# graphdeco-inria/gaussian-splatting

Measured on AMD Instinct MI355X. Metric: Mpix/s forward (1 M Gaussians @1080p); train iters/s alongside, higher is better.
Workload: dtype f32; 1 GPU; configs[1] stand-in: 1M random Gaussians (SURVEY 8(d) generator, seed 0, s_med 0.012), 1920x1080 forward render, SH degree 3; P=1000000, visible=876281, num_rendered=7916318, tiles=8160, parallelism=one GPU, mode=single, render_fwd_variant=0, options=, frame_streams=1

## Files before the change

### gaussian-splatting_amd/csrc/preprocess.hip

```cpp
#include "gsr_internal.h"
#include "gsr_adam_math.h"
#include "gsr_frame.h"

namespace {

#ifndef GSR_PRE_OCC_FWD
#define GSR_PRE_OCC_FWD
#endif
#ifndef GSR_PRE_OCC_BWD
#ifdef GSR_SIMT_SHIM
#define GSR_PRE_OCC_BWD
#else
#define GSR_PRE_OCC_BWD __attribute__((amdgpu_waves_per_eu(2, 2)))
#endif
#endif

constexpr int SH_ROW = 52;

__device__ __forceinline__ void load_cam(const GsrCamDev& c, GsrCam& cam) {
    cam.W = c.W; cam.H = c.H; cam.gx = c.gx; cam.gy = c.gy;
    cam.focal_x = c.focal_x; cam.focal_y = c.focal_y; cam.limx = c.limx; cam.limy = c.limy;
    cam.scale_modifier = c.scale_modifier; cam.sh_degree = c.sh_degree; cam.M = c.M;
    cam.antialiasing = c.antialiasing; cam.tile_y0 = c.tile_y0; cam.tile_y1 = c.tile_y1; cam.snug = c.snug;
#pragma unroll
    for (int i = 0; i < 16; ++i) { cam.view[i] = c.view[i]; cam.proj[i] = c.proj[i]; }
#pragma unroll
    for (int i = 0; i < 3; ++i) cam.campos[i] = c.campos[i];
}

#ifdef GSR_SIMT_SHIM
__device__ __forceinline__ void fence_loaded12(float4 (&)[12]) {}
#else
typedef float gsr_v4f __attribute__((ext_vector_type(4)));
__device__ __forceinline__ void fence_loaded12(float4 (&v)[12]) {
    gsr_v4f r[12];
#pragma unroll
    for (int k = 0; k < 12; ++k) r[k] = (gsr_v4f){v[k].x, v[k].y, v[k].z, v[k].w};
    asm volatile("" : "+v"(r[0]), "+v"(r[1]), "+v"(r[2]), "+v"(r[3]), "+v"(r[4]), "+v"(r[5]), "+v"(r[6]), "+v"(r[7]), "+v"(r[8]),
                      "+v"(r[9]), "+v"(r[10]), "+v"(r[11]));
#pragma unroll
    for (int k = 0; k < 12; ++k) v[k] = make_float4(r[k].x, r[k].y, r[k].z, r[k].w);
    __builtin_amdgcn_sched_barrier(0);
}
#endif

__device__ __forceinline__ void wave_load_sh16(const float* __restrict__ shs, int64_t i0, int P, uint64_t rows, int lane,
                                               float* tile) {
    const float4* src = reinterpret_cast<const float4*>(shs + i0 * 48);
    float4 v[12];
#pragma unroll
    for (int it = 0; it < 12; ++it) {
        const int idx = it * 64 + lane;
        const int g = idx / 12;
        v[it] = src[(((rows >> g) & 1ull) && i0 + g < P) ? idx : 0];
    }
    fence_loaded12(v);
#pragma unroll
    for (int it = 0; it < 12; ++it) {
        const int idx = it * 64 + lane;
        const int g = idx / 12, part = idx - g * 12;
        *reinterpret_cast<float4*>(tile + g * SH_ROW + part * 4) = v[it];
    }
    __builtin_amdgcn_wave_barrier();
}
__device__ __forceinline__ void wave_issue_sh16(const float* __restrict__ shs, int64_t i0, int P, int lane, float4 (&reg)[12]) {
    const float4* src = reinterpret_cast<const float4*>(shs + i0 * 48);
#pragma unroll
    for (int it = 0; it < 12; ++it) {
        const int idx = it * 64 + lane;
        const int g = idx / 12;
        reg[it] = (i0 + g < P) ? src[idx] : make_float4(0.f, 0.f, 0.f, 0.f);
    }
}
__device__ __forceinline__ void wave_commit_sh16(const float4 (&reg)[12], uint64_t rows, int lane, float* tile) {
#pragma unroll
    for (int it = 0; it < 12; ++it) {
        const int idx = it * 64 + lane;
        const int g = idx / 12, part = idx - g * 12;
        if ((rows >> g) & 1ull) *reinterpret_cast<float4*>(tile + g * SH_ROW + part * 4) = reg[it];
    }
    __builtin_amdgcn_wave_barrier();
}
__device__ __forceinline__ void wave_store_sh16(float* __restrict__ dst_all, int64_t i0, int P, int lane, const float* tile) {
    float4* dst = reinterpret_cast<float4*>(dst_all + i0 * 48);
    __builtin_amdgcn_wave_barrier();
#pragma unroll
    for (int it = 0; it < 12; ++it) {
        const int idx = it * 64 + lane;
        const int g = idx / 12, part = idx - g * 12;
        if (i0 + g < P) dst[idx] = *reinterpret_cast<const float4*>(tile + g * SH_ROW + part * 4);
    }
    __builtin_amdgcn_wave_barrier();
}

constexpr int SPLIT_DC = 64 * 45;
__device__ __forceinline__ void wave_load_sh_split_dense(const float* __restrict__ dc, const float* __restrict__ rest, int64_t i0,
                                                         int P, uint64_t rows, int lane, float* tile) {
    const int nrow = (int)((P - i0) < 64 ? (P - i0) : 64);
    const float* src = rest + i0 * 45;
    const float* sdc = dc + i0 * 3;
    const int nrest = nrow * 45, ndc = nrow * 3;
    float4 v[12];
    bool ok[12];
#pragma unroll
    for (int it = 0; it < 12; ++it) {
        const int f = (it * 64 + lane) * 4;
        const int g0 = f / 45, g1 = (f + 3) / 45;
        const bool want = rows == ~0ull || ((((rows >> (g0 & 63)) | (rows >> (g1 & 63))) & 1ull) != 0);
        ok[it] = want && f + 3 < nrest;
        v[it] = *reinterpret_cast<const float4*>(src + (ok[it] ? f : 0));
    }
    const int fd = lane * 4;
    const bool okd = rows != 0ull && fd + 3 < ndc;
    const float4 vd = *reinterpret_cast<const float4*>(sdc + (okd ? fd : 0));
    fence_loaded12(v);
#pragma unroll
    for (int it = 0; it < 12; ++it) {
        const int f = (it * 64 + lane) * 4;
        *reinterpret_cast<float4*>(tile + (f < 64 * 45 ? f : 64 * 48 + lane * 4)) = v[it];
    }
    *reinterpret_cast<float4*>(tile + (fd < 64 * 3 ? SPLIT_DC + fd : 64 * 48 + lane * 4)) = vd;
    (void)ok; (void)okd;
    if (lane < (nrest & 3)) tile[(nrest & ~3) + lane] = src[(nrest & ~3) + lane];
    if (lane < (ndc & 3)) tile[SPLIT_DC + (ndc & ~3) + lane] = sdc[(ndc & ~3) + lane];
    __builtin_amdgcn_wave_barrier();
}
__device__ __forceinline__ void wave_store_sh_split_dense(float* __restrict__ d_dc, float* __restrict__ d_rest, int64_t i0, int P,
                                                          int lane, const float* tile) {
    const int nrow = (int)((P - i0) < 64 ? (P - i0) : 64);
    float* dst = d_rest + i0 * 45;
    const int nrest = nrow * 45;
    __builtin_amdgcn_wave_barrier();
#pragma unroll
    for (int it = 0; it < 12; ++it) {
        const int f = (it * 64 + lane) * 4;
        if (f + 3 < nrest) {
            *reinterpret_cast<float4*>(dst + f) = *reinterpret_cast<const float4*>(tile + f);
        } else if (f < nrest) {
            for (int c = 0; c < 3; ++c)
                if (f + c < nrest) dst[f + c] = tile[f + c];
        }
    }
    float* ddc = d_dc + i0 * 3;
    const int ndc = nrow * 3, fd = lane * 4;
    if (fd + 3 < ndc) {
        *reinterpret_cast<float4*>(ddc + fd) = *reinterpret_cast<const float4*>(tile + SPLIT_DC + fd);
    } else if (fd < ndc) {
        for (int c = 0; c < 3; ++c)
            if (fd + c < ndc) ddc[fd + c] = tile[SPLIT_DC + fd + c];
    }
    __builtin_amdgcn_wave_barrier();
}
template <bool SPLIT>
__global__ void __launch_bounds__(256) GSR_PRE_OCC_FWD
preprocess_fwd_kernel(GsrCamDev camd, int P, const float* __restrict__ means3D, const float* __restrict__ shs,
                      const float* __restrict__ colors_precomp, const float* __restrict__ opacities,
                      const float* __restrict__ scales, const float* __restrict__ rotations,
                      const float* __restrict__ cov3D_precomp, float4* __restrict__ splats,
                      uint2* __restrict__ rect, uint32_t* __restrict__ tiles, uint32_t* __restrict__ clamped_out,
                      uint32_t* __restrict__ keys, uint32_t* __restrict__ vals, int32_t* __restrict__ radii,
                      GsrFrameStatsDev fs) {
    __shared__ __attribute__((aligned(16))) float s_sh[4][64 * SH_ROW];
    GsrCam cam;
    load_cam(camd, cam);
    const int lane = threadIdx.x & 63, wv = threadIdx.x >> 6;
    float* tile = s_sh[wv];
    const float* dc = SPLIT ? camd.sh_dc : nullptr;
    const bool staged_sh = shs != nullptr && cam.M == 16;
    const bool speculative = (cam.tile_y1 - cam.tile_y0) * 4 >= cam.gy;
    GsrFrameAcc acc;
    for (int64_t i0 = ((int64_t)blockIdx.x * blockDim.x + threadIdx.x) - lane; i0 < P; i0 += (int64_t)gridDim.x * blockDim.x) {
        const int64_t i = i0 + lane;
        const bool in_range = i < P;
        GsrSplat sp;
        sp.radius = 0; sp.tiles = 0; sp.minx = sp.miny = sp.maxx = sp.maxy = 0; sp.depth = 0.f;
        float mean[3] = {0.f, 0.f, 0.f};
        bool vis = false;
        const bool spec_sh = staged_sh && speculative;
        float4 g_rot = make_float4(0.f, 0.f, 0.f, 0.f);
        float g_s[3] = {0.f, 0.f, 0.f}, g_op = 0.f;
        if (spec_sh) {
            float4 shreg[12];
            if (!SPLIT) wave_issue_sh16(shs, i0, P, lane, shreg);
            if (in_range) {
                mean[0] = means3D[i * 3 + 0]; mean[1] = means3D[i * 3 + 1]; mean[2] = means3D[i * 3 + 2];
                g_op = opacities[i];
                if (!cov3D_precomp) {
                    g_s[0] = scales[i * 3 + 0]; g_s[1] = scales[i * 3 + 1]; g_s[2] = scales[i * 3 + 2];
                    g_rot = reinterpret_cast<const float4*>(rotations)[i];
                }
            }
            if (SPLIT) wave_load_sh_split_dense(dc, shs, i0, P, ~0ull, lane, tile);
            else wave_commit_sh16(shreg, ~0ull, lane, tile);
        }
        if (in_range) {
            if (!spec_sh) {
                mean[0] = means3D[i * 3 + 0]; mean[1] = means3D[i * 3 + 1]; mean[2] = means3D[i * 3 + 2];
                g_op = opacities[i];
            }
            float cov[6];
            if (cov3D_precomp) {
#pragma unroll
                for (int k = 0; k < 6; ++k) cov[k] = cov3D_precomp[i * 6 + k];
            } else {
                if (!spec_sh) {
                    g_s[0] = scales[i * 3 + 0]; g_s[1] = scales[i * 3 + 1]; g_s[2] = scales[i * 3 + 2];
                    g_rot = reinterpret_cast<const float4*>(rotations)[i];
                }
                const float q[4] = {g_rot.x, g_rot.y, g_rot.z, g_rot.w};
                gsr_cov3d(g_s, cam.scale_modifier, q, cov);
            }
            vis = gsr_project(cam, mean, cov, g_op, sp);
        }
        const bool need_color = vis && sp.tiles > 0;
        if (staged_sh) {
            const uint64_t rows = __ballot(need_color);
            if (rows) {
                if (spec_sh) {  }
                else if (SPLIT) wave_load_sh_split_dense(dc, shs, i0, P, rows, lane, tile);
                else wave_load_sh16(shs, i0, P, rows, lane, tile);
            }
        }
        if (!in_range) continue;
        uint32_t clampbits = 0;
        float4 q0 = make_float4(0.f, 0.f, 0.f, 0.f), q1 = q0, q2 = q0;
        if (vis) {
            float rgb[3] = {0.f, 0.f, 0.f};
            if (!need_color) {
            } else if (colors_precomp) {
                rgb[0] = colors_precomp[i * 3 + 0]; rgb[1] = colors_precomp[i * 3 + 1]; rgb[2] = colors_precomp[i * 3 + 2];
            } else if (staged_sh) {
                if (SPLIT) gsr_sh_to_rgb_row(cam.sh_degree, 16, GsrShRowSplit{tile + SPLIT_DC + lane * 3, tile + lane * 45}, mean, cam.campos, rgb, clampbits);
                else gsr_sh_to_rgb_row(cam.sh_degree, 16, GsrShRowAligned{tile + lane * SH_ROW}, mean, cam.campos, rgb, clampbits);
            } else if (!SPLIT) {
                gsr_sh_to_rgb(cam.sh_degree, cam.M, shs + i * (int64_t)cam.M * 3, mean, cam.campos, rgb, clampbits);
            }
            q0 = make_float4(sp.px, sp.py, sp.conA, sp.conB);
            q1 = make_float4(sp.conC, sp.opacity, rgb[0], rgb[1]);
            q2 = make_float4(rgb[2], sp.depth, sp.tau, gsr_inv_depth(sp.depth));
        }
        const uint2 rc = make_uint2(sp.minx | (sp.maxx << 16), sp.miny | (sp.maxy << 16));
        splats[i * 4 + 0] = q0;
        splats[i * 4 + 1] = q1;
        splats[i * 4 + 2] = q2;
        splats[i * 4 + 3] = make_float4(__uint_as_float(rc.x), __uint_as_float(rc.y), 0.f, __uint_as_float(sp.tiles));
        rect[i] = rc;
        tiles[i] = sp.tiles;
        if (clamped_out) clamped_out[i] = clampbits;
        radii[i] = sp.radius;
        const uint32_t key = gsr_depth_key(sp.depth, sp.tiles != 0u, acc.ovf);
        keys[i] = key;
        vals[i] = (uint32_t)i;
        acc.add(key, sp.tiles);
    }
    gsr_frame_stats_commit(fs, acc.tiles, acc.kmin, acc.kmax, acc.ovf);
}


__device__ __forceinline__ void adam_piece(float4& p, const float4& g, float4& m, float4& v, const float (&a)[6], int sparse, bool k0, bool k1,
                                           bool k2, bool k3) {
    if (sparse) {
        if (k0) gsr_sparse_adam1(p.x, g.x, m.x, v.x, a[0], a[1], a[2], a[3], a[4], a[5]);
        if (k1) gsr_sparse_adam1(p.y, g.y, m.y, v.y, a[0], a[1], a[2], a[3], a[4], a[5]);
        if (k2) gsr_sparse_adam1(p.z, g.z, m.z, v.z, a[0], a[1], a[2], a[3], a[4], a[5]);
        if (k3) gsr_sparse_adam1(p.w, g.w, m.w, v.w, a[0], a[1], a[2], a[3], a[4], a[5]);
    } else {
        gsr_adam1(p.x, g.x, m.x, v.x, a[0], a[1], a[2], a[3], a[4], a[5]);
        gsr_adam1(p.y, g.y, m.y, v.y, a[0], a[1], a[2], a[3], a[4], a[5]);
        gsr_adam1(p.z, g.z, m.z, v.z, a[0], a[1], a[2], a[3], a[4], a[5]);
        gsr_adam1(p.w, g.w, m.w, v.w, a[0], a[1], a[2], a[3], a[4], a[5]);
    }
}
__device__ __forceinline__ void wave_adam_sh_split_dense(const GsrShAdamDev& ad, int64_t i0, int P, uint64_t rows, int lane, const float* tile) {
    const int nrow = (int)((P - i0) < 64 ? (P - i0) : 64);
    const int nrest = nrow * 45, ndc = nrow * 3;
    float* pr = ad.rest + i0 * 45; float* mr = ad.rest_m + i0 * 45; float* vr = ad.rest_v + i0 * 45;
    __builtin_amdgcn_wave_barrier();
#pragma unroll 1
    for (int it0 = 0; it0 < 12; it0 += 4) {
        float4 pp[4], mm[4], vv[4];
#pragma unroll
        for (int k = 0; k < 4; ++k) {
            const int f = ((it0 + k) * 64 + lane) * 4;
            const int fo = f + 3 < nrest ? f : 0;
            pp[k] = *reinterpret_cast<const float4*>(pr + fo);
            mm[k] = *reinterpret_cast<const float4*>(mr + fo);
            vv[k] = *reinterpret_cast<const float4*>(vr + fo);
        }
#pragma unroll
        for (int k = 0; k < 4; ++k) {
            const int f = ((it0 + k) * 64 + lane) * 4;
            if (f + 3 < nrest) {
                const float4 g = *reinterpret_cast<const float4*>(tile + f);
                const int r0 = f / 45, r1 = (f + 1) / 45, r2 = (f + 2) / 45, r3 = (f + 3) / 45;
                adam_piece(pp[k], g, mm[k], vv[k], ad.rest_a, ad.sparse, (rows >> r0) & 1ull, (rows >> r1) & 1ull, (rows >> r2) & 1ull,
                           (rows >> r3) & 1ull);
                *reinterpret_cast<float4*>(pr + f) = pp[k];
                *reinterpret_cast<float4*>(mr + f) = mm[k];
                *reinterpret_cast<float4*>(vr + f) = vv[k];
            } else if (f < nrest) {
                for (int c = 0; c < 3; ++c)
                    if (f + c < nrest && ((rows >> ((f + c) / 45)) & 1ull)) {
                        float p1 = pr[f + c], m1 = mr[f + c], v1 = vr[f + c];
                        if (ad.sparse) gsr_sparse_adam1(p1, tile[f + c], m1, v1, ad.rest_a[0], ad.rest_a[1], ad.rest_a[2], ad.rest_a[3], ad.rest_a[4], ad.rest_a[5]);
                        else gsr_adam1(p1, tile[f + c], m1, v1, ad.rest_a[0], ad.rest_a[1], ad.rest_a[2], ad.rest_a[3], ad.rest_a[4], ad.rest_a[5]);
                        pr[f + c] = p1; mr[f + c] = m1; vr[f + c] = v1;
                    }
            }
        }
    }
    float* pd = ad.dc + i0 * 3; float* md = ad.dc_m + i0 * 3; float* vd = ad.dc_v + i0 * 3;
    const int fd = lane * 4;
    if (fd + 3 < ndc) {
        float4 p4 = *reinterpret_cast<const float4*>(pd + fd), m4 = *reinterpret_cast<const float4*>(md + fd), v4 = *reinterpret_cast<const float4*>(vd + fd);
        const float4 g = *reinterpret_cast<const float4*>(tile + SPLIT_DC + fd);
        adam_piece(p4, g, m4, v4, ad.dc_a, ad.sparse, (rows >> (fd / 3)) & 1ull, (rows >> ((fd + 1) / 3)) & 1ull, (rows >> ((fd + 2) / 3)) & 1ull,
                   (rows >> ((fd + 3) / 3)) & 1ull);
        *reinterpret_cast<float4*>(pd + fd) = p4;
        *reinterpret_cast<float4*>(md + fd) = m4;
        *reinterpret_cast<float4*>(vd + fd) = v4;
    } else if (fd < ndc) {
        for (int c = 0; c < 3; ++c)
            if (fd + c < ndc && ((rows >> ((fd + c) / 3)) & 1ull)) {
                float p1 = pd[fd + c], m1 = md[fd + c], v1 = vd[fd + c];
                if (ad.sparse) gsr_sparse_adam1(p1, tile[SPLIT_DC + fd + c], m1, v1, ad.dc_a[0], ad.dc_a[1], ad.dc_a[2], ad.dc_a[3], ad.dc_a[4], ad.dc_a[5]);
                else gsr_adam1(p1, tile[SPLIT_DC + fd + c], m1, v1, ad.dc_a[0], ad.dc_a[1], ad.dc_a[2], ad.dc_a[3], ad.dc_a[4], ad.dc_a[5]);
                pd[fd + c] = p1; md[fd + c] = m1; vd[fd + c] = v1;
            }
    }
    __builtin_amdgcn_wave_barrier();
}

constexpr int GSR_CAM_TERMS = 27;
__device__ __forceinline__ double shfl_xor_f64(double v, int m) {
    uint64_t u;
    __builtin_memcpy(&u, &v, 8);
    const uint32_t lo = __shfl_xor((uint32_t)u, m), hi = __shfl_xor((uint32_t)(u >> 32), m);
    u = ((uint64_t)hi << 32) | lo;
    __builtin_memcpy(&v, &u, 8);
    return v;
}
constexpr int CAM_ROW = 17;
__device__ __forceinline__ double wave_column_sum16(const float* t, int lane) {
    __builtin_amdgcn_wave_barrier();
    const int c = lane & 15, r0 = (lane >> 4) * 16;
    double s = (double)t[r0 * CAM_ROW + c];
#pragma unroll
    for (int k = 1; k < 16; ++k) s = s + (double)t[(r0 + k) * CAM_ROW + c];
    __builtin_amdgcn_wave_barrier();
    s = s + shfl_xor_f64(s, 16);
    return s + shfl_xor_f64(s, 32);
}
struct GsrCamPartialsDev {
    double* partials;
};
template <bool CAM> struct GsrBwdTail { typedef GsrShAdamDev type; };
template <> struct GsrBwdTail<true> { typedef GsrCamPartialsDev type; };

template <bool SPLIT, bool ADAM = false, bool CAM = false>
__global__ void __launch_bounds__(256) GSR_PRE_OCC_BWD
preprocess_bwd_kernel(GsrCamDev camd, int P, const float* __restrict__ means3D, const float* shs,
                      const float* __restrict__ colors_precomp, const float* __restrict__ opacities,
                      const float* __restrict__ scales, const float* __restrict__ rotations,
                      const float* __restrict__ cov3D_precomp, const int32_t* __restrict__ radii,
                      const uint32_t* __restrict__ clamped, const float4* __restrict__ grads,
                      float* __restrict__ dL_dmeans2D, float* __restrict__ dL_dcolors, float* __restrict__ dL_dopacity,
                      float* __restrict__ dL_dmeans3D, float* __restrict__ dL_dcov3D, float* __restrict__ dL_dsh,
                      float* __restrict__ dL_dscales, float* __restrict__ dL_drotations, typename GsrBwdTail<CAM>::type adam) {
    static_assert(!(ADAM && CAM), "the fused SH Adam step and the camera gradient are not combined");
    __shared__ __attribute__((aligned(16))) float s_sh[4][64 * SH_ROW];
    __shared__ float s_cam[CAM ? 4 : 1][CAM ? 64 * CAM_ROW : 1];
    GsrCam cam;
    load_cam(camd, cam);
    const int M = cam.M;
    const int lane = threadIdx.x & 63, wv = threadIdx.x >> 6;
    float* tile = s_sh[wv];
    const float* dc = SPLIT ? camd.sh_dc : nullptr;
    float* dL_ddc = SPLIT ? camd.dL_dsh_dc : nullptr;
    const bool staged_sh = shs != nullptr && M == 16;
    constexpr int sh_row = SH_ROW;
    double cam_acc_v = 0.0, cam_acc_p = 0.0;
    for (int64_t i0 = ((int64_t)blockIdx.x * blockDim.x + threadIdx.x) - lane; i0 < P; i0 += (int64_t)gridDim.x * blockDim.x) {
        const int64_t i = i0 + lane;
        const bool in_range = i < P;
        [[maybe_unused]] float ddir[3] = {0.f, 0.f, 0.f};
        float dmean[3] = {0.f, 0.f, 0.f};
        float dcov[6] = {0.f, 0.f, 0.f, 0.f, 0.f, 0.f};
        float dscale[3] = {0.f, 0.f, 0.f};
        float drot[4] = {0.f, 0.f, 0.f, 0.f};
        float dop = 0.f;
        float dm2x = 0.f, dm2y = 0.f;
        float drgb[3] = {0.f, 0.f, 0.f};
        int rad = 0;
        float4 g0 = make_float4(0.f, 0.f, 0.f, 0.f), g1 = g0, g2 = g0, q4 = g0;
        float mean[3] = {0.f, 0.f, 0.f}, s[3] = {0.f, 0.f, 0.f}, q[4], cov[6], op_in = 0.f;
        if (in_range) {
            rad = radii[i];
            g0 = grads[i * 3 + 0]; g1 = grads[i * 3 + 1]; g2 = grads[i * 3 + 2];
            mean[0] = means3D[i * 3 + 0]; mean[1] = means3D[i * 3 + 1]; mean[2] = means3D[i * 3 + 2];
            op_in = opacities[i];
            if (cov3D_precomp) {
#pragma unroll
                for (int k = 0; k < 6; ++k) cov[k] = cov3D_precomp[i * 6 + k];
            } else {
                s[0] = scales[i * 3 + 0]; s[1] = scales[i * 3 + 1]; s[2] = scales[i * 3 + 2];
                q4 = reinterpret_cast<const float4*>(rotations)[i];
            }
        }
        if (staged_sh) {
            if (SPLIT) wave_load_sh_split_dense(dc, shs, i0, P, ~0ull, lane, tile);
            else wave_load_sh16(shs, i0, P, ~0ull, lane, tile);
        }
        const bool vis = in_range && rad > 0;
        if (vis) {
            GsrSplatGrad g;
            g.dpx = g0.x; g.dpy = g0.y; g.dconA = g0.z; g.dconB = g0.w;
            g.dconC = g1.x; g.dopacity = g1.y; g.dr = g1.z; g.dg = g1.w;
            g.db = g2.x; g.dinvdepth = g2.y;
            drgb[0] = g.dr; drgb[1] = g.dg; drgb[2] = g.db;
            GsrBwdReal covr[6], dcovr[6] = {0, 0, 0, 0, 0, 0};
            if (!cov3D_precomp) {
                q[0] = q4.x; q[1] = q4.y; q[2] = q4.z; q[3] = q4.w;
                gsr_cov3d_r<GsrBwdReal>(s, cam.scale_modifier, q, covr);
            } else {
#pragma unroll
                for (int k = 0; k < 6; ++k) covr[k] = cov[k];
            }
            if constexpr (CAM) {
                gsr_project_backward_r<GsrBwdReal>(cam, mean, covr, op_in, g, dmean, dcovr, dop,
                                                   reinterpret_cast<GsrProjTerms*>(s_cam[wv] + lane * CAM_ROW));
            } else {
                gsr_project_backward_r<GsrBwdReal>(cam, mean, covr, op_in, g, dmean, dcovr, dop);
            }
            dm2x = g.dpx * (0.5f * (float)cam.W);
            dm2y = g.dpy * (0.5f * (float)cam.H);
            if (!cov3D_precomp) gsr_cov3d_backward_r<GsrBwdReal>(s, cam.scale_modifier, q, dcovr, dscale, drot);
#pragma unroll
            for (int k = 0; k < 6; ++k) dcov[k] = (float)dcovr[k];
        }
        if (vis) {
            if (shs) {
                float rgb_unused[3];
                uint32_t clampbits = 0;
                if (staged_sh) {
                    if (SPLIT) {
                        const GsrShRowSplit row{tile + SPLIT_DC + lane * 3, tile + lane * 45};
                        gsr_sh_to_rgb_row(cam.sh_degree, 16, row, mean, cam.campos, rgb_unused, clampbits);
                        gsr_sh_backward_row(cam.sh_degree, 16, row, mean, cam.campos, clampbits, drgb,
                                            GsrShRowSplitOut{tile + SPLIT_DC + lane * 3, tile + lane * 45}, dmean, CAM ? ddir : nullptr);
                    } else {
                        const GsrShRowAligned row{tile + lane * sh_row};
                        gsr_sh_to_rgb_row(cam.sh_degree, 16, row, mean, cam.campos, rgb_unused, clampbits);
                        gsr_sh_backward_row(cam.sh_degree, 16, row, mean, cam.campos, clampbits, drgb,
                                            GsrShRowAlignedOut{tile + lane * sh_row}, dmean, CAM ? ddir : nullptr);
                    }
                } else if (!SPLIT) {
                    gsr_sh_to_rgb(cam.sh_degree, M, shs + i * (int64_t)M * 3, mean, cam.campos, rgb_unused, clampbits);
                    gsr_sh_backward_row(cam.sh_degree, M, GsrShRow{shs + i * (int64_t)M * 3}, mean, cam.campos, clampbits, drgb,
                                        GsrShRowOut{dL_dsh + i * (int64_t)M * 3}, dmean, CAM ? ddir : nullptr);
                }
            }
        } else if (shs) {
            if (staged_sh) {
#pragma unroll
                for (int k = 0; k < 12; ++k) {
                    if (SPLIT) {
                        if (k < 11) {
                            tile[lane * 45 + k * 4 + 0] = 0.f; tile[lane * 45 + k * 4 + 1] = 0.f;
                            tile[lane * 45 + k * 4 + 2] = 0.f; tile[lane * 45 + k * 4 + 3] = 0.f;
                        } else {
                            tile[lane * 45 + 44] = 0.f;
                            tile[SPLIT_DC + lane * 3 + 0] = 0.f; tile[SPLIT_DC + lane * 3 + 1] = 0.f; tile[SPLIT_DC + lane * 3 + 2] = 0.f;
                        }
                    } else {
                        *reinterpret_cast<float4*>(tile + lane * sh_row + k * 4) = make_float4(0.f, 0.f, 0.f, 0.f);
                    }
                }
            } else if (in_range && !SPLIT) {
                float* o = dL_dsh + i * (int64_t)M * 3;
                for (int k = 0; k < M * 3; ++k) o[k] = 0.f;
            }
        }
        if (staged_sh) {
            if constexpr (SPLIT && ADAM) wave_adam_sh_split_dense(adam, i0, P, adam.sparse ? __ballot(vis) : ~0ull, lane, tile);
            else if (SPLIT) wave_store_sh_split_dense(dL_ddc, dL_dsh, i0, P, lane, tile);
            else wave_store_sh16(dL_dsh, i0, P, lane, tile);
        }
        if constexpr (CAM) {
            float* rowp = s_cam[wv] + lane * CAM_ROW;
            float dtf[3], dhf[3], w[9];
#pragma unroll
            for (int r = 0; r < 3; ++r) { dtf[r] = vis ? rowp[r] : 0.f; dhf[r] = vis ? rowp[12 + r] : 0.f; }
#pragma unroll
            for (int k = 0; k < 9; ++k) w[k] = vis ? rowp[3 + k] : 0.f;
            const double p[3] = {(double)mean[0], (double)mean[1], (double)mean[2]};
#pragma unroll
            for (int j = 0; j < 3; ++j)
#pragma unroll
                for (int r = 0; r < 3; ++r) rowp[3 * j + r] = (float)((double)dtf[r] * p[j] + (double)w[3 * j + r]);
#pragma unroll
            for (int r = 0; r < 3; ++r) {
                rowp[9 + r] = dtf[r];
                rowp[12 + r] = ddir[r];
            }
            rowp[15] = 0.f;
            cam_acc_v += wave_column_sum16(s_cam[wv], lane);
#pragma unroll
            for (int r = 0; r < 3; ++r) {
#pragma unroll
                for (int j = 0; j < 3; ++j) rowp[3 * j + r] = (float)((double)dhf[r] * p[j]);
                rowp[9 + r] = dhf[r];
            }
            rowp[12] = rowp[13] = rowp[14] = 0.f;
            cam_acc_p += wave_column_sum16(s_cam[wv], lane);
        }
        if (!in_range) continue;
        dL_dmeans2D[i * 3 + 0] = dm2x; dL_dmeans2D[i * 3 + 1] = dm2y; dL_dmeans2D[i * 3 + 2] = 0.f;
        if (dL_dcolors) { dL_dcolors[i * 3 + 0] = drgb[0]; dL_dcolors[i * 3 + 1] = drgb[1]; dL_dcolors[i * 3 + 2] = drgb[2]; }
        dL_dopacity[i] = dop;
        dL_dmeans3D[i * 3 + 0] = dmean[0]; dL_dmeans3D[i * 3 + 1] = dmean[1]; dL_dmeans3D[i * 3 + 2] = dmean[2];
#pragma unroll
        for (int k = 0; k < 6; ++k)
            if (dL_dcov3D) dL_dcov3D[i * 6 + k] = dcov[k];
        if (dL_dscales) {
            dL_dscales[i * 3 + 0] = dscale[0]; dL_dscales[i * 3 + 1] = dscale[1]; dL_dscales[i * 3 + 2] = dscale[2];
            reinterpret_cast<float4*>(dL_drotations)[i] = make_float4(drot[0], drot[1], drot[2], drot[3]);
        }
    }
    if constexpr (CAM) {
        __syncthreads();
        double* red = reinterpret_cast<double*>(&s_sh[0][0]);
        const int c = lane;
        if (c < 15) red[wv * 32 + (c < 12 ? c : c + 12)] = cam_acc_v;
        if (c < 12) red[wv * 32 + 12 + c] = cam_acc_p;
        __syncthreads();
        const int t = threadIdx.x;
        if (t < GSR_CAM_TERMS) adam.partials[(int64_t)t * gridDim.x + blockIdx.x] = ((red[t] + red[32 + t]) + red[64 + t]) + red[96 + t];
    }
}

__global__ void __launch_bounds__(256)
camera_grad_finish_kernel(const double* __restrict__ partials, int rows, float* __restrict__ dview, float* __restrict__ dproj,
                          float* __restrict__ dcampos) {
    __shared__ double red[GSR_CAM_TERMS][257];
    const int t = threadIdx.x;
    static_assert(GSR_CAM_MAX_ROWS <= 4 * 256, "camera_grad_finish_kernel sums at most four rows per thread");
#pragma unroll
    for (int c = 0; c < GSR_CAM_TERMS; ++c) {
        double v[4];
#pragma unroll
        for (int k = 0; k < 4; ++k) {
            const int r = t + 256 * k;
            v[k] = partials[(int64_t)c * rows + (r < rows ? r : 0)];
        }
        double s = 0.0;
#pragma unroll
        for (int k = 0; k < 4; ++k) s = s + (t + 256 * k < rows ? v[k] : 0.0);
        red[c][t] = s;
    }
    __syncthreads();
    if (t < GSR_CAM_TERMS) {
        double s = 0.0;
        for (int k = 0; k < 256; ++k) s += red[t][k];
        if (t < 12) {
            dview[t % 3 + 4 * (t / 3)] = (float)s;
        } else if (t < 24) {
            const int c = t - 12, row = c % 3 == 2 ? 3 : c % 3;
            dproj[row + 4 * (c / 3)] = (float)s;
        } else {
            dcampos[t - 24] = (float)(-s);
        }
    }
    if (t < 4) {
        dview[3 + 4 * t] = 0.f;
        dproj[2 + 4 * t] = 0.f;
    }
}

__global__ void __launch_bounds__(256)
mark_visible_kernel(int P, const float* __restrict__ means3D, const float* __restrict__ vm, uint8_t* __restrict__ present) {
    for (int64_t i = (int64_t)blockIdx.x * blockDim.x + threadIdx.x; i < P; i += (int64_t)gridDim.x * blockDim.x) {
        const float x = means3D[i * 3 + 0], y = means3D[i * 3 + 1], z = means3D[i * 3 + 2];
        const float pvz = vm[2] * x + vm[6] * y + vm[10] * z + vm[14];
        present[i] = pvz > GSR_NEAR_Z ? 1 : 0;
    }
}

int g_stream_grid_cap = 1024;

inline int stream_grid(int64_t n) {
    int64_t b = (n + 255) / 256;
    if (b > g_stream_grid_cap) b = g_stream_grid_cap;
    if (b < 1) b = 1;
    return (int)b;
}

}

int gsr_launch_preprocess(const GsrCamDev& cam, int P, const float* means3D, const float* shs,
                          const float* colors_precomp, const float* opacities, const float* scales,
                          const float* rotations, const float* cov3D_precomp, GsrGeom g, int32_t* radii,
                          const GsrFrameStatsDev& fs, hipStream_t st) {
    const int grid = stream_grid(P) < GSR_FRAME_MAX_GROUPS ? stream_grid(P) : GSR_FRAME_MAX_GROUPS;
#define GSR_PRE_FWD(SPLIT_)                                                                                                            \
    hipLaunchKernelGGL((preprocess_fwd_kernel<SPLIT_>), dim3(grid), dim3(256), 0, st, cam, P, means3D, shs, colors_precomp,              \
                       opacities, scales, rotations, cov3D_precomp, g.splats, g.rect, g.tiles,                                         \
                        nullptr, g.keys[0], g.vals[0], radii, fs)
    if (cam.sh_dc) GSR_PRE_FWD(true);
    else GSR_PRE_FWD(false);
#undef GSR_PRE_FWD
    return grid;
}

void gsr_launch_preprocess_backward(const GsrCamDev& cam, int P, const float* means3D, const float* shs,
                                    const float* colors_precomp, const float* opacities, const float* scales,
                                    const float* rotations, const float* cov3D_precomp, const int32_t* radii,
                                    GsrGeom g, const float* splat_grads, float* dL_dmeans2D, float* dL_dcolors,
                                    float* dL_dopacity, float* dL_dmeans3D, float* dL_dcov3D, float* dL_dsh,
                                    float* dL_dscales, float* dL_drotations, hipStream_t st, const GsrCamGradDev* camg) {
#define GSR_PRE_BWD(SPLIT_)                                                                                                     \
    hipLaunchKernelGGL((preprocess_bwd_kernel<SPLIT_>), dim3(stream_grid(P)), dim3(256), 0, st, cam, P, means3D, shs,             \
                       colors_precomp, opacities, scales, rotations, cov3D_precomp, radii, g.clamped,                                 \
                       reinterpret_cast<const float4*>(splat_grads), dL_dmeans2D, dL_dcolors, dL_dopacity, dL_dmeans3D, dL_dcov3D,     \
                       dL_dsh, dL_dscales, dL_drotations, GsrShAdamDev{})
#define GSR_PRE_BWD_CAM(SPLIT_)                                                                                                 \
    hipLaunchKernelGGL((preprocess_bwd_kernel<SPLIT_, false, true>), dim3(grid), dim3(256), 0, st, cam, P, means3D, shs,          \
                       colors_precomp, opacities, scales, rotations, cov3D_precomp, radii, g.clamped,                                 \
                       reinterpret_cast<const float4*>(splat_grads), dL_dmeans2D, dL_dcolors, dL_dopacity, dL_dmeans3D, dL_dcov3D,     \
                       dL_dsh, dL_dscales, dL_drotations, GsrCamPartialsDev{camg->partials})
    if (camg) {
        const int grid = stream_grid(P) < (int)gsr_camera_grad_rows(P) ? stream_grid(P) : (int)gsr_camera_grad_rows(P);
        if (cam.sh_dc) GSR_PRE_BWD_CAM(true);
        else GSR_PRE_BWD_CAM(false);
        hipLaunchKernelGGL(camera_grad_finish_kernel, dim3(1), dim3(256), 0, st, (const double*)camg->partials, grid, camg->dview,
                           camg->dproj, camg->dcampos);
        return;
    }
    if (cam.sh_dc) GSR_PRE_BWD(true);
    else GSR_PRE_BWD(false);
#undef GSR_PRE_BWD
#undef GSR_PRE_BWD_CAM
}

size_t gsr_camera_grad_rows(int P) {
    const int64_t b = ((int64_t)(P > 0 ? P : 0) + 255) / 256;
    return (size_t)(b < 1 ? 1 : (b > GSR_CAM_MAX_ROWS ? GSR_CAM_MAX_ROWS : b));
}

void gsr_launch_preprocess_backward_sh_adam(const GsrCamDev& cam, int P, const float* means3D, const float* opacities,
                                            const float* scales, const float* rotations, const float* cov3D_precomp,
                                            const int32_t* radii, GsrGeom g, const float* splat_grads, float* dL_dmeans2D,
                                            float* dL_dopacity, float* dL_dmeans3D, float* dL_dcov3D, float* dL_dscales,
                                            float* dL_drotations, const GsrShAdamDev& adam, hipStream_t st) {
    hipLaunchKernelGGL((preprocess_bwd_kernel<true, true>), dim3(stream_grid(P)), dim3(256), 0, st, cam, P, means3D,
                       (const float*)adam.rest, (const float*)nullptr, opacities, scales, rotations, cov3D_precomp, radii, g.clamped,
                       reinterpret_cast<const float4*>(splat_grads), dL_dmeans2D, (float*)nullptr, dL_dopacity, dL_dmeans3D, dL_dcov3D,
                       (float*)nullptr, dL_dscales, dL_drotations, adam);
}

void gsr_launch_mark_visible(int P, const float* means3D, const float* view, uint8_t* present, hipStream_t st) {
    hipLaunchKernelGGL(mark_visible_kernel, dim3(stream_grid(P)), dim3(256), 0, st, P, means3D, view, present);
}


void gsr_set_preprocess_grid_cap(int cap) { g_stream_grid_cap = cap < 64 ? 64 : cap; }
```

Measured before the change: 6105 Mpix/s.

## Software-pipeline preprocess loads and stage SH coefficients via global-to-LDS DMA

Rewrites the preprocess forward loop so each wave prefetches the next iteration's Gaussian attributes into registers. It also issues direct global-to-LDS loads (global_load_lds) for the next batch of SH coefficients while the current batch is projected and shaded. The SH tile loses its padded row stride so the DMA layout stays contiguous, and the split dc/rest layout handles ragged tails with a separate scalar fixup. The intent is to hide memory latency and drop the register round-trip for SH staging. In exchange the code carries more live registers and relies on an explicit waitcnt encoding, and the unpadded LDS rows may cause bank conflicts.

```diff
diff --git a/gaussian-splatting_amd/csrc/preprocess.hip b/gaussian-splatting_amd/csrc/preprocess.hip
--- a/gaussian-splatting_amd/csrc/preprocess.hip
+++ b/gaussian-splatting_amd/csrc/preprocess.hip
@@ -63,24 +63,6 @@
     }
     __builtin_amdgcn_wave_barrier();
 }
-__device__ __forceinline__ void wave_issue_sh16(const float* __restrict__ shs, int64_t i0, int P, int lane, float4 (&reg)[12]) {
-    const float4* src = reinterpret_cast<const float4*>(shs + i0 * 48);
-#pragma unroll
-    for (int it = 0; it < 12; ++it) {
-        const int idx = it * 64 + lane;
-        const int g = idx / 12;
-        reg[it] = (i0 + g < P) ? src[idx] : make_float4(0.f, 0.f, 0.f, 0.f);
-    }
-}
-__device__ __forceinline__ void wave_commit_sh16(const float4 (&reg)[12], uint64_t rows, int lane, float* tile) {
-#pragma unroll
-    for (int it = 0; it < 12; ++it) {
-        const int idx = it * 64 + lane;
-        const int g = idx / 12, part = idx - g * 12;
-        if ((rows >> g) & 1ull) *reinterpret_cast<float4*>(tile + g * SH_ROW + part * 4) = reg[it];
-    }
-    __builtin_amdgcn_wave_barrier();
-}
 __device__ __forceinline__ void wave_store_sh16(float* __restrict__ dst_all, int64_t i0, int P, int lane, const float* tile) {
     float4* dst = reinterpret_cast<float4*>(dst_all + i0 * 48);
     __builtin_amdgcn_wave_barrier();
@@ -151,6 +133,99 @@
     }
     __builtin_amdgcn_wave_barrier();
 }
+constexpr int SH_TILE = 64 * 48;
+#ifdef GSR_SIMT_SHIM
+__device__ __forceinline__ void lds_dma16(const float* src, float* lds, int lane) {
+    *reinterpret_cast<float4*>(lds + lane * 4) = *reinterpret_cast<const float4*>(src);
+}
+#else
+__device__ __forceinline__ void lds_dma16(const float* src, float* lds, int) {
+    __builtin_amdgcn_global_load_lds((const __attribute__((address_space(1))) void*)src, (__attribute__((address_space(3))) void*)lds, 16, 0, 0);
+}
+#endif
+#ifdef GSR_SIMT_SHIM
+__device__ __forceinline__ void wait_sh_copy() {}
+__device__ __forceinline__ void fence_f(float&) {}
+#else
+__device__ __forceinline__ void wait_sh_copy() { __builtin_amdgcn_s_waitcnt(0x0f70); }
+__device__ __forceinline__ void fence_f(float& v) { asm volatile("" : "+v"(v)); }
+#endif
+__device__ __forceinline__ void wave_dma_sh16(const float* __restrict__ shs, int64_t i0, int P, uint64_t rows, int lane, float* tile) {
+    const float* src = shs + i0 * 48;
+#pragma unroll
+    for (int it = 0; it < 12; ++it) {
+        const int s = it * 64 + lane, g = s / 12;
+        lds_dma16(src + ((((rows >> g) & 1ull) && i0 + g < P) ? s * 4 : 0), tile + it * 256, lane);
+    }
+}
+__device__ __forceinline__ void wave_dma_sh_split(const float* __restrict__ dc, const float* __restrict__ rest, int64_t i0, int P, uint64_t rows,
+                                                  int lane, float* tile) {
+    const int nrow = (int)((P - i0) < 64 ? (P - i0) : 64);
+    const int nrest = nrow * 45, ndc = nrow * 3;
+    const float* src = rest + i0 * 45;
+    const float* sdc = dc + i0 * 3;
+#pragma unroll
+    for (int it = 0; it < 12; ++it) {
+        const int s = it * 64 + lane;
+        const float* p = src;
+        if (s < 720) {
+            const int f = s * 4, g0 = f / 45, g1 = (f + 3) / 45;
+            const bool want = rows == ~0ull || ((((rows >> (g0 & 63)) | (rows >> (g1 & 63))) & 1ull) != 0);
+            if (want && f + 3 < nrest) p = src + f;
+        } else {
+            const int fd = (s - 720) * 4, g0 = fd / 3, g1 = (fd + 3) / 3;
+            const bool want = rows == ~0ull || ((((rows >> (g0 & 63)) | (rows >> (g1 & 63))) & 1ull) != 0);
+            if (want && fd + 3 < ndc) p = sdc + fd;
+        }
+        lds_dma16(p, tile + it * 256, lane);
+    }
+}
+struct GsrShRagged {
+    int at;
+    float v;
+};
+__device__ __forceinline__ GsrShRagged sh_split_ragged_load(const float* __restrict__ dc, const float* __restrict__ rest, int64_t i0, int P,
+                                                            int lane) {
+    const int nrow = (int)((P - i0) < 64 ? (P - i0) : 64);
+    const int nrest = nrow * 45, ndc = nrow * 3;
+    const bool in_dc = lane >= 4;
+    const int f = (in_dc ? ndc & ~3 : nrest & ~3) + (lane & 3);
+    GsrShRagged r{-1, 0.f};
+    if (lane < 8 && (lane & 3) < (in_dc ? ndc & 3 : nrest & 3)) {
+        r.at = (in_dc ? SPLIT_DC : 0) + f;
+        r.v = in_dc ? dc[i0 * 3 + f] : rest[i0 * 45 + f];
+        fence_f(r.v);
+    }
+    return r;
+}
+
+struct GsrFwdIn {
+    float mean[3], op, p[7];
+};
+__device__ __forceinline__ GsrFwdIn load_fwd_in(int64_t i, int P, const float* __restrict__ means3D, const float* __restrict__ opacities,
+                                                const float* __restrict__ scales, const float* __restrict__ rotations,
+                                                const float* __restrict__ cov3D_precomp) {
+    const int64_t j = i < P ? i : P - 1;
+    GsrFwdIn g;
+    g.mean[0] = means3D[j * 3 + 0]; g.mean[1] = means3D[j * 3 + 1]; g.mean[2] = means3D[j * 3 + 2];
+    g.op = opacities[j];
+    if (cov3D_precomp) {
+#pragma unroll
+        for (int k = 0; k < 6; ++k) g.p[k] = cov3D_precomp[j * 6 + k];
+        g.p[6] = 0.f;
+    } else {
+        g.p[0] = scales[j * 3 + 0]; g.p[1] = scales[j * 3 + 1]; g.p[2] = scales[j * 3 + 2];
+        const float4 r = reinterpret_cast<const float4*>(rotations)[j];
+        g.p[3] = r.x; g.p[4] = r.y; g.p[5] = r.z; g.p[6] = r.w;
+    }
+    return g;
+}
+__device__ __forceinline__ void fence_fwd_in(GsrFwdIn& g) {
+    fence_f(g.mean[0]); fence_f(g.mean[1]); fence_f(g.mean[2]); fence_f(g.op);
+#pragma unroll
+    for (int k = 0; k < 7; ++k) fence_f(g.p[k]);
+}
+
 template <bool SPLIT>
 __global__ void __launch_bounds__(256) GSR_PRE_OCC_FWD
 preprocess_fwd_kernel(GsrCamDev camd, int P, const float* __restrict__ means3D, const float* __restrict__ shs,
@@ -160,7 +235,7 @@
                       uint2* __restrict__ rect, uint32_t* __restrict__ tiles, uint32_t* __restrict__ clamped_out,
                       uint32_t* __restrict__ keys, uint32_t* __restrict__ vals, int32_t* __restrict__ radii,
                       GsrFrameStatsDev fs) {
-    __shared__ __attribute__((aligned(16))) float s_sh[4][64 * SH_ROW];
+    __shared__ __attribute__((aligned(16))) float s_sh[4][SH_TILE];
     GsrCam cam;
     load_cam(camd, cam);
     const int lane = threadIdx.x & 63, wv = threadIdx.x >> 6;
@@ -168,60 +243,55 @@
     const float* dc = SPLIT ? camd.sh_dc : nullptr;
     const bool staged_sh = shs != nullptr && cam.M == 16;
     const bool speculative = (cam.tile_y1 - cam.tile_y0) * 4 >= cam.gy;
+    const bool spec_sh = staged_sh && speculative;
+    const int64_t stride = (int64_t)gridDim.x * blockDim.x;
+    int64_t i0 = ((int64_t)blockIdx.x * blockDim.x + threadIdx.x) - lane;
+    GsrFwdIn nxt = {};
+    if (i0 < P) {
+        nxt = load_fwd_in(i0 + lane, P, means3D, opacities, scales, rotations, cov3D_precomp);
+        fence_fwd_in(nxt);
+        if (spec_sh) {
+            if (SPLIT) wave_dma_sh_split(dc, shs, i0, P, ~0ull, lane, tile);
+            else wave_dma_sh16(shs, i0, P, ~0ull, lane, tile);
+        }
+    }
     GsrFrameAcc acc;
-    for (int64_t i0 = ((int64_t)blockIdx.x * blockDim.x + threadIdx.x) - lane; i0 < P; i0 += (int64_t)gridDim.x * blockDim.x) {
+    for (; i0 < P; i0 += stride) {
         const int64_t i = i0 + lane;
         const bool in_range = i < P;
+        const int64_t i0n = i0 + stride < P ? i0 + stride : i0;
+        const GsrFwdIn in = nxt;
+        nxt = load_fwd_in(i0n + lane, P, means3D, opacities, scales, rotations, cov3D_precomp);
         GsrSplat sp;
         sp.radius = 0; sp.tiles = 0; sp.minx = sp.miny = sp.maxx = sp.maxy = 0; sp.depth = 0.f;
-        float mean[3] = {0.f, 0.f, 0.f};
         bool vis = false;
-        const bool spec_sh = staged_sh && speculative;
-        float4 g_rot = make_float4(0.f, 0.f, 0.f, 0.f);
-        float g_s[3] = {0.f, 0.f, 0.f}, g_op = 0.f;
-        if (spec_sh) {
-            float4 shreg[12];
-            if (!SPLIT) wave_issue_sh16(shs, i0, P, lane, shreg);
-            if (in_range) {
-                mean[0] = means3D[i * 3 + 0]; mean[1] = means3D[i * 3 + 1]; mean[2] = means3D[i * 3 + 2];
-                g_op = opacities[i];
-                if (!cov3D_precomp) {
-                    g_s[0] = scales[i * 3 + 0]; g_s[1] = scales[i * 3 + 1]; g_s[2] = scales[i * 3 + 2];
-                    g_rot = reinterpret_cast<const float4*>(rotations)[i];
-                }
-            }
-            if (SPLIT) wave_load_sh_split_dense(dc, shs, i0, P, ~0ull, lane, tile);
-            else wave_commit_sh16(shreg, ~0ull, lane, tile);
-        }
         if (in_range) {
-            if (!spec_sh) {
-                mean[0] = means3D[i * 3 + 0]; mean[1] = means3D[i * 3 + 1]; mean[2] = means3D[i * 3 + 2];
-                g_op = opacities[i];
-            }
             float cov[6];
             if (cov3D_precomp) {
 #pragma unroll
-                for (int k = 0; k < 6; ++k) cov[k] = cov3D_precomp[i * 6 + k];
+                for (int k = 0; k < 6; ++k) cov[k] = in.p[k];
             } else {
-                if (!spec_sh) {
-                    g_s[0] = scales[i * 3 + 0]; g_s[1] = scales[i * 3 + 1]; g_s[2] = scales[i * 3 + 2];
-                    g_rot = reinterpret_cast<const float4*>(rotations)[i];
-                }
-                const float q[4] = {g_rot.x, g_rot.y, g_rot.z, g_rot.w};
-                gsr_cov3d(g_s, cam.scale_modifier, q, cov);
-            }
-            vis = gsr_project(cam, mean, cov, g_op, sp);
+                gsr_cov3d(in.p, cam.scale_modifier, in.p + 3, cov);
+            }
+            vis = gsr_project(cam, in.mean, cov, in.op, sp);
         }
         const bool need_color = vis && sp.tiles > 0;
-        if (staged_sh) {
+        if (staged_sh && !spec_sh) {
             const uint64_t rows = __ballot(need_color);
             if (rows) {
-                if (spec_sh) {  }
-                else if (SPLIT) wave_load_sh_split_dense(dc, shs, i0, P, rows, lane, tile);
-                else wave_load_sh16(shs, i0, P, rows, lane, tile);
-            }
-        }
-        if (!in_range) continue;
+                if (SPLIT) wave_dma_sh_split(dc, shs, i0, P, rows, lane, tile);
+                else wave_dma_sh16(shs, i0, P, rows, lane, tile);
+            }
+        }
+        const GsrShRagged rg = SPLIT && staged_sh ? sh_split_ragged_load(dc, shs, i0, P, lane) : GsrShRagged{-1, 0.f};
+        wait_sh_copy();
+        if (staged_sh) {
+            __builtin_amdgcn_wave_barrier();
+            if (SPLIT) {
+                if (rg.at >= 0) tile[rg.at] = rg.v;
+                __builtin_amdgcn_wave_barrier();
+            }
+        }
         uint32_t clampbits = 0;
         float4 q0 = make_float4(0.f, 0.f, 0.f, 0.f), q1 = q0, q2 = q0;
         if (vis) {
@@ -230,15 +300,22 @@
             } else if (colors_precomp) {
                 rgb[0] = colors_precomp[i * 3 + 0]; rgb[1] = colors_precomp[i * 3 + 1]; rgb[2] = colors_precomp[i * 3 + 2];
             } else if (staged_sh) {
-                if (SPLIT) gsr_sh_to_rgb_row(cam.sh_degree, 16, GsrShRowSplit{tile + SPLIT_DC + lane * 3, tile + lane * 45}, mean, cam.campos, rgb, clampbits);
-                else gsr_sh_to_rgb_row(cam.sh_degree, 16, GsrShRowAligned{tile + lane * SH_ROW}, mean, cam.campos, rgb, clampbits);
+                if (SPLIT) gsr_sh_to_rgb_row(cam.sh_degree, 16, GsrShRowSplit{tile + SPLIT_DC + lane * 3, tile + lane * 45}, in.mean, cam.campos, rgb, clampbits);
+                else gsr_sh_to_rgb_row(cam.sh_degree, 16, GsrShRowAligned{tile + lane * 48}, in.mean, cam.campos, rgb, clampbits);
             } else if (!SPLIT) {
-                gsr_sh_to_rgb(cam.sh_degree, cam.M, shs + i * (int64_t)cam.M * 3, mean, cam.campos, rgb, clampbits);
+                gsr_sh_to_rgb(cam.sh_degree, cam.M, shs + i * (int64_t)cam.M * 3, in.mean, cam.campos, rgb, clampbits);
             }
             q0 = make_float4(sp.px, sp.py, sp.conA, sp.conB);
             q1 = make_float4(sp.conC, sp.opacity, rgb[0], rgb[1]);
             q2 = make_float4(rgb[2], sp.depth, sp.tau, gsr_inv_depth(sp.depth));
         }
+        fence_fwd_in(nxt);
+        if (spec_sh) {
+            __builtin_amdgcn_wave_barrier();
+            if (SPLIT) wave_dma_sh_split(dc, shs, i0n, P, ~0ull, lane, tile);
+            else wave_dma_sh16(shs, i0n, P, ~0ull, lane, tile);
+        }
+        if (!in_range) continue;
         const uint2 rc = make_uint2(sp.minx | (sp.maxx << 16), sp.miny | (sp.maxy << 16));
         splats[i * 4 + 0] = q0;
         splats[i * 4 + 1] = q1;
@@ -253,6 +330,7 @@
         vals[i] = (uint32_t)i;
         acc.add(key, sp.tiles);
     }
+    if (spec_sh) wait_sh_copy();
     gsr_frame_stats_commit(fs, acc.tiles, acc.kmin, acc.kmax, acc.ovf);
 }
 
```

Result: no change. 6147 Mpix/s (median of 6 runs) (+0.7%).
